# NSLab-CUK/LiteralKG

Measured on AMD Instinct MI355X. Metric: kg_edges_aggregated_per_sec, higher is better.
Workload: dtype f32

## Files before the change

literalkg_amd/_native.py:

```python
import ctypes as C
import os

_LIB_PATH = os.path.join(os.path.dirname(os.path.abspath(__file__)), "lib", "liblkg_hip.so")
_lib = None

i64, i32, f32, vp, u64 = C.c_int64, C.c_int32, C.c_float, C.c_void_p, C.c_uint64

PROTOTYPES = {
    "lkg_version": [],
    "lkg_last_error": [],
    "lkg_preload": [],
    "lkg_csr_build": [i64, i64, vp, vp, vp, vp, vp, vp, vp, vp, vp],
    "lkg_csr_transpose": [i64, i64, i64, vp, vp, vp, vp, vp],
    "lkg_row_partition": [i64, vp, i32, vp],
    "lkg_csr_coo_indices_i64": [i64, i64, vp, vp, vp, vp],
    "lkg_csr_build_device_workspace": [i64, i64],
    "lkg_csr_build_device": [i64, i64, vp, vp, vp, vp, vp, vp, vp, vp, vp, vp, i64, vp],
    "lkg_csr_transpose_device_workspace": [i64, i64],
    "lkg_csr_transpose_device": [i64, i64, i64, vp, vp, vp, vp, vp, vp, i64, vp],
    "lkg_triples_count": [C.c_char_p, vp],
    "lkg_triples_read": [C.c_char_p, i64, vp, vp, vp, vp],
    "lkg_triples_dedup": [i64, vp, vp, vp, vp, vp],
    "lkg_laplacian_f32": [i64, i64, i64, vp, vp, vp, vp, i32, vp],
    "lkg_laplacian_device_f32": [i64, i64, i32, vp, vp, vp, vp, i32, vp, vp, vp],
# ... 115 lines not shown
TRAIN_PROTOTYPES = {
    "lkg_nssa_fwd_f32": [i64, i64, i32, vp, i64, vp, i64, vp, i64, i32, f32, f32, f32, vp, vp, vp, vp, vp],
    "lkg_nssa_bwd_f32": [i64, i64, i32, vp, i64, vp, i64, vp, i64, i32, f32, vp, vp, vp, vp, vp, i64, vp, i64, vp, i64, vp],
}
SAMPLE_PROTOTYPES = {
    "lkg_sample_negatives": [i64, i64, u64, i64, vp, vp, vp, i64, i64, i32, i32, i32, vp, vp, vp, vp, vp, vp, vp, vp, vp, vp,
                             vp, i64, vp, i64, vp, vp, vp, vp],
    "lkg_relation_cardinality": [i64, i64, i64, vp, vp, vp, i64, vp, vp, vp, vp, vp, vp, vp],
    "lkg_answer_counts": [i64, vp, vp, vp, i64, vp, vp, vp, vp, vp, vp, vp, vp, vp],
}
RELATION_TRAIN_PROTOTYPES = {
    "lkg_relation_loss_fwd_f32": [i64, i32, i32, vp, i64, i64, vp, i64, vp, vp, vp, vp, vp, vp, vp, f32, vp, i64, vp, vp, vp],
    "lkg_relation_loss_bwd_f32": [i64, i32, i32, vp, i64, i64, vp, i64, vp, f32, vp, vp, i64, vp, i64, vp, i64, vp],
}
ORDERED_GEMM_PROTOTYPES = {
    "lkg_gemm_ordered_splits": [i32, i32, i64, i64, i64],
    "lkg_gemm_ordered_partition": [i64, i32, vp],
    "lkg_gemm_ordered_workspace": [i64, i64, i64, i32],
    "lkg_gemm_ordered_f32": [i32, i32, i64, i64, i64, i32, f32, vp, i64, vp, i64, f32, vp, i64, vp, vp, i64, vp],
}
NEIGHBOR_PROTOTYPES = {
    "lkg_csr_sample_rows": [i64, vp, vp, vp, vp, i32, u64, u64, i32, vp, vp, vp, vp],
}
_PAIR_ACCEPT_HEAD = [i64, i64, vp, vp, vp, vp, vp, vp, vp, vp, vp, vp, vp, vp, vp, vp, i32, vp]
PAIR_ACCEPT_PROTOTYPES = {
    "lkg_pair_mlp_accept_count_f32": _PAIR_ACCEPT_HEAD + [vp],
    "lkg_pair_mlp_accept_append_f32": _PAIR_ACCEPT_HEAD + [i64, vp, vp, vp, vp, vp],
    "lkg_pair_mlp_accept_emit_f32": _PAIR_ACCEPT_HEAD + [vp, vp, vp, vp, vp, vp, vp],
}
LIST_PROTOTYPES = {
    "lkg_list_scores_f32": [i64, i64, i64, i32, vp, i64, vp, vp, i64, vp, vp, i64, i32, vp, i64, vp],
    "lkg_list_count_f32": [i64, i64, i64, i32, vp, i64, vp, i64, vp, vp, i64, vp, vp, vp, vp, vp, vp, vp, vp, vp, vp, vp, vp],
}
_RESTYPE = {"lkg_last_error": C.c_char_p, "lkg_csr_build_device_workspace": C.c_int64,
            "lkg_gemm_tall_workspace": C.c_int64, "lkg_gemm_workspace": C.c_int64,
            "lkg_linear_act_layernorm_workspace": C.c_int64, "lkg_narrow_layer_bwd_workspace": C.c_int64,
            "lkg_csr_transpose_device_workspace": C.c_int64, "lkg_binary_curve_workspace": C.c_int64,
            "lkg_threshold_fit_workspace": C.c_int64, "lkg_accept_order_workspace": C.c_int64,
            "lkg_gemm_ordered_splits": C.c_int32, "lkg_gemm_ordered_partition": C.c_int64,
            "lkg_gemm_ordered_workspace": C.c_int64}


class LkgError(RuntimeError):
    pass


def lib_path():
    return _LIB_PATH


def load():
    global _lib
    if _lib is not None:
        return _lib
    if not os.path.exists(_LIB_PATH):
        raise LkgError(
            f"{_LIB_PATH} is missing: the HIP extension has not been built. Run "
            "`python -c 'import __graft_entry__ as g; g.build()'` (or `python -m literalkg_amd.build`). "
            "literalkg_amd has no CPU fallback.")
    lib = C.CDLL(_LIB_PATH)
    for name, argtypes in list(PROTOTYPES.items()) + list(EXTRA_PROTOTYPES.items()) + list(TRAIN_PROTOTYPES.items()) + \
            list(SAMPLE_PROTOTYPES.items()) + list(RELATION_TRAIN_PROTOTYPES.items()) + \
            list(ORDERED_GEMM_PROTOTYPES.items()) + list(NEIGHBOR_PROTOTYPES.items()) + \
            list(PAIR_ACCEPT_PROTOTYPES.items()) + list(LIST_PROTOTYPES.items()):
        fn = getattr(lib, name)
        fn.argtypes = argtypes
        fn.restype = _RESTYPE.get(name, C.c_int)
    _lib = lib
    return lib


_preloaded = False


def preload():
    global _preloaded
    if _preloaded:
        return
    import torch
    if not torch.cuda.is_initialized():
        return
    _preloaded = True
    lib = load()
    if lib.lkg_preload() != 0:
        msg = lib.lkg_last_error()
        raise LkgError(f"lkg_preload failed: {msg.decode() if msg else '?'}")


def call(name, *args):
    lib = load()
    if not _preloaded:
        preload()
    rc = getattr(lib, name)(*args)
    if rc != 0:
        msg = lib.lkg_last_error()
        raise LkgError(f"{name} failed ({rc}): {msg.decode() if msg else '?'}")

# ... 18 lines not shown
```

literalkg_amd/build.py:

```python
import hashlib
import os
import shutil
import subprocess
import sys
from concurrent.futures import ThreadPoolExecutor

HERE = os.path.dirname(os.path.abspath(__file__))
CSRC = os.path.join(HERE, "csrc")
LIB = os.path.join(HERE, "lib", "liblkg_hip.so")
OBJ = os.path.join(HERE, "lib", "obj")
SOURCES = ["lkg_graph_host.cpp", "lkg_spmm.hip", "lkg_attention.hip", "lkg_score.hip", "lkg_rowwise.hip",
           "lkg_gemm.hip", "lkg_batch.hip", "lkg_csr_device.hip", "lkg_gemm_tall.hip", "lkg_gemm_wgrad.hip", "lkg_layer.hip",
           "lkg_rank.hip", "lkg_topk.hip", "lkg_pairmlp.hip", "lkg_triples.hip", "lkg_relations.hip",
           "lkg_accept.hip", "lkg_retrieval.hip", "lkg_softmax.hip", "lkg_kvsall.hip", "lkg_nssa.hip", "lkg_negatives.hip",
           "lkg_relation_loss.hip", "lkg_gemm_ordered.hip", "lkg_neighbors.hip", "lkg_lists.hip"]
FLAGS = ["-O3", "--offload-arch=gfx950", "-fPIC", "-std=c++17"]


def _headers():
    return [os.path.join(CSRC, f) for f in sorted(os.listdir(CSRC)) if f.endswith(".h")] + \
           [os.path.join(HERE, "..", "include", h) for h in ("literalkg_hip.h", "literalkg_hip_ext.h", "literalkg_hip_train.h",
                                                                "literalkg_hip_sample.h", "literalkg_hip_relation_train.h",
                                                                "literalkg_hip_gemm_ordered.h", "literalkg_hip_neighbors.h",
                                                                "literalkg_hip_pair_accept.h", "literalkg_hip_lists.h")]


TAG_FILE = os.path.join(HERE, "lib", "flags.tag")


def _stale(tag):
    if not os.path.exists(LIB):
        return True
    if os.path.exists(TAG_FILE) and open(TAG_FILE).read().strip() != tag:
        return True
    t = os.path.getmtime(LIB)
    deps = [os.path.join(CSRC, f) for f in os.listdir(CSRC)] + _headers()
    return any(os.path.getmtime(d) > t for d in deps)


def _flag_tag(extra):
    return hashlib.sha256(" ".join(FLAGS + extra).encode()).hexdigest()[:12]


def build(force=False, verbose=True):
    extra = os.environ.get("LKG_EXTRA_HIPCC_FLAGS", "").split()
    tag = _flag_tag(extra)
    if not force and not _stale(tag):
        return LIB
    hipcc = shutil.which("hipcc") or "/opt/rocm/bin/hipcc"
    if not os.path.exists(hipcc):
        raise RuntimeError("hipcc not found: cannot build literalkg_amd/lib/liblkg_hip.so")
    os.makedirs(OBJ, exist_ok=True)
    newest_header = max(os.path.getmtime(h) for h in _headers())
    todo, objs = [], []
    for s in SOURCES:
        src = os.path.join(CSRC, s)
        obj = os.path.join(OBJ, f"{os.path.splitext(s)[0]}.{tag}.o")
# ... 27 lines not shown
```

literalkg_amd/csrc/lkg_graph_host.cpp:

```cpp
#include <fcntl.h>
#include <sys/mman.h>
#include <sys/stat.h>
#include <unistd.h>

#include <algorithm>
#include <atomic>
#include <cerrno>
#include <cmath>
#include <cstdlib>
#include <cstring>
#include <new>
#include <thread>
#include <vector>

#include "lkg_common.h"

static thread_local char g_err[512] = "";

void lkg_set_error(const char *fmt, ...) {
    va_list ap;
    va_start(ap, fmt);
    vsnprintf(g_err, sizeof(g_err), fmt, ap);
    va_end(ap);
}

extern "C" const char *lkg_last_error(void) { return g_err; }
extern "C" int lkg_version(void) { return 100;  }

int lkg_internal_preload_spmm();
int lkg_internal_preload_attention();
int lkg_internal_preload_batch();
int lkg_internal_preload_csr_device();
int lkg_internal_preload_gemm();
int lkg_internal_preload_gemm_tall();
int lkg_internal_preload_gemm_wgrad();
int lkg_internal_preload_rowwise();
int lkg_internal_preload_score();
int lkg_internal_preload_layer();
int lkg_internal_preload_rank();
int lkg_internal_preload_topk();
int lkg_internal_preload_pairmlp();
int lkg_internal_preload_triples();
int lkg_internal_preload_relations();
int lkg_internal_preload_accept();
int lkg_internal_preload_retrieval();
int lkg_internal_preload_softmax();
int lkg_internal_preload_kvsall();
int lkg_internal_preload_nssa();
int lkg_internal_preload_negatives();
int lkg_internal_preload_relation_loss();
int lkg_internal_preload_gemm_ordered();
int lkg_internal_preload_neighbors();
int lkg_internal_preload_lists();

extern "C" int lkg_preload(void) {
    const int failed = lkg_internal_preload_spmm() + lkg_internal_preload_attention() + lkg_internal_preload_batch() + lkg_internal_preload_csr_device() + lkg_internal_preload_gemm() + lkg_internal_preload_gemm_tall() + lkg_internal_preload_gemm_wgrad() + lkg_internal_preload_rowwise() + lkg_internal_preload_score() + lkg_internal_preload_layer() + lkg_internal_preload_rank() + lkg_internal_preload_topk() + lkg_internal_preload_pairmlp() + lkg_internal_preload_triples() + lkg_internal_preload_relations() + lkg_internal_preload_accept() + lkg_internal_preload_retrieval() + lkg_internal_preload_softmax() + lkg_internal_preload_kvsall() + lkg_internal_preload_nssa() + lkg_internal_preload_negatives() + lkg_internal_preload_relation_loss() + lkg_internal_preload_gemm_ordered() + lkg_internal_preload_neighbors() + lkg_internal_preload_lists();
    if (failed) {
        lkg_set_error("lkg_preload: %d of the library's code objects could not be loaded on the current device", failed);
        return LKG_ERR_HIP;
    }
    return LKG_OK;
}

namespace {
template <class F>
void parallel_rows(int64_t n, F &&fn) {
    unsigned hw = std::thread::hardware_concurrency();
    int nt = (int)std::min<int64_t>(std::max(1u, std::min(hw, 32u)), std::max<int64_t>(1, n / 65536));
    if (nt <= 1) {
        fn(0, n);
        return;
    }
    std::vector<std::thread> th;
    int64_t step = (n + nt - 1) / nt;
    for (int i = 0; i < nt; ++i) {
        int64_t lo = i * step, hi = std::min(n, lo + step);
        if (lo < hi) th.emplace_back([=, &fn] { fn(lo, hi); });
    }
    for (auto &x : th) x.join();
}
}

extern "C" int lkg_csr_build(int64_t n_entities, int64_t n_edges, const int64_t *h,
                             const int64_t *t, const int64_t *r, int32_t *rowptr, int32_t *col,
                             int32_t *eptr, int32_t *rel, int64_t *order, int64_t *nnz_out) {
    LKG_REQUIRE(n_entities >= 0 && n_entities < INT32_MAX, "lkg_csr_build: n_entities %lld out of int32 range",
                (long long)n_entities);
    LKG_REQUIRE(n_edges >= 0 && n_edges < INT32_MAX, "lkg_csr_build: n_edges %lld out of int32 range",
                (long long)n_edges);
// ... 383 lines not shown
```

literalkg_amd/model.py:

```python
from __future__ import annotations

import math
import os
from typing import Optional

import torch
import torch.nn as nn

from . import ops, pruned
from .gate import Gate, GateMul
from .graph import KGStructure


class AttentionCSR:

    def __init__(self, graph: KGStructure, val: torch.Tensor, val_t: Optional[torch.Tensor] = None):
        self.graph = graph
        self.val = val
        self.val_t = val_t if val_t is not None else (
            ops.permute_values(val, graph.t_perm) if graph.t_perm is not None and val.is_cuda else None)

    def aggregate(self, ego: torch.Tensor, plus_self: bool = False, bias: Optional[torch.Tensor] = None) -> torch.Tensor:
        return ops.aggregate(ego, self.graph, self.val, self.val_t, plus_self, bias)

# ... 123 lines not shown
    def narrows(self) -> bool:
        return self.aggregator_type == "gcn" and not self.use_residual and 2 * self.out_dim <= self.in_dim

    def forward(self, ego_embeddings, A_in: AttentionCSR, all_layers, lamda, alpha, l):
        ego = ego_embeddings
        h0 = all_layers[0]
        kind = self.aggregator_type
        if kind == "gcn":
            att = getattr(A_in, "att", A_in)
            if self.narrows() and isinstance(att, AttentionCSR):
                p = ops.linear(ego, self.linear.weight, None)
                return self._finish(att.aggregate(p, True, bias=self.linear.bias))
            if not self.use_residual:
                return self._linear_finish((A_in.aggregate(ego, True),), (self.linear.weight,), self.linear.bias)
            z = self._res_lin(self.linear, A_in.aggregate(ego, True), h0, lamda, alpha, l)
            return self._finish(z)
        if kind == "gin":
            return self._gin(ego, A_in.aggregate(ego, True), h0, all_layers, lamda, alpha, l)
        side = A_in.aggregate(ego)
        if kind == "graphsage":
            if self.use_residual:
                wh = self.linear_h.weight
                hi = ops.multi_linear((ego, side), (wh[:, :self.in_dim], wh[:, self.in_dim:]), self.linear_h.bias)
                z = self._res_lin(self.linear, hi, h0, lamda, alpha, l)
            else:
                w = self.linear.weight
                return self._linear_finish((ego, side), (w[:, :self.in_dim], w[:, self.in_dim:]), self.linear.bias)
            return self._finish(z)
        if kind == "bi-interaction":
            h0p = None
            if self.use_residual:
                h0p = self.h0_projection if self.h0_projection is not None else \
                    ops.linear(h0, self.linear_h0.weight, self.linear_h0.bias)
            ms, mp = ops.bi_mix(ego, side, h0p, alpha)
            if self.use_residual:
                wp = self._identity_map(lamda, l)
                s, b = self._lin_mapped(self.linear1, ms, wp), self._lin_mapped(self.linear2, mp, wp)
            else:
                s, b = self._lin(self.linear1, ms), self._lin(self.linear2, mp)
            return self._finish(ops.leaky_relu_sum(b, s), slope=1.0)
        raise NotImplementedError(kind)

    def _gin(self, ego, ego_plus_side, h0, all_layers, lamda, alpha, l):
        if self.num_layers == 1:
            raise AttributeError("gin with n_mlp_layers == 1 cannot run in the reference either "
                                 "(inp_linear/out_linear are never created, model.py:66-68, 133)")
        stack = self._lin(self.inp_linear, ego)
        h = self._lin(self.inp_linear, ego_plus_side)
        for lin, norm in zip(self.linears, self.mlp_layer_norms):
            h, _ = ops.act_layernorm(self._lin(lin, h), norm.weight, norm.bias, want_norm=False)
            stack = ops.axpby(stack, h)
        z = self._res_lin(self.out_linear, stack, h0, lamda, alpha, l)
        if len(all_layers) > 1:
            return self._finish(z, extra_sum=list(all_layers[1:]))
        return self._finish(z)


class LiteralKG(nn.Module):

    def __init__(self, args, n_entities, n_relations, A_in=None, numerical_literals=None, text_literals=None,
                 scoring: str = "transr"):
        super().__init__()
        if scoring not in ("transr", "transe"):
            raise ValueError(scoring)
        self.scoring = scoring
        self.args = args
# ... 593 lines not shown
```

literalkg_amd/ops.py:

```python
from __future__ import annotations

from typing import Optional, Sequence, Tuple

import torch
from torch.autograd import Function

from . import _native as N
from .graph import KGStructure, LONG_ROW_THRESHOLD

LEAKY_SLOPE = 0.01
LN_EPS = 1e-5
NORMALIZE_EPS = 1e-12


_raw_stream = getattr(torch._C, "_cuda_getCurrentRawStream", None)


def _stream():
    if _raw_stream is not None:
        return _raw_stream(torch.cuda.current_device())
    return torch.cuda.current_stream().cuda_stream


def _need_gpu(*ts):
# ... 1346 lines not shown
        rows_n, rows_y = tagged_rows(gyn), tagged_rows(gy)
        rows = union_rows(rows_y, rows_n) if (gy is None or rows_y is not None) and (gyn is None or rows_n is not None) else None
        gy_ = _f32_rows(gy) if gy is not None else None
        gyn_ = _f32_rows(gyn) if gyn is not None else None
        fused = (not rows_worth_compacting(rows, n) and need[0] and need[1] and gamma.data_ptr() % 16 == 0
                 and N.load().lkg_narrow_layer_bwd_ok(n, x.shape[1], d, N.ptr(x), _ld(x), N.ptr(z), _ld(z), N.ptr(y),
                                                      _ld(y) if y is not None else 0, N.ptr(gy_), _ld(gy_) if gy_ is not None else 0,
                                                      N.ptr(gyn_), _ld(gyn_) if gyn_ is not None else 0))
        if not fused:
            gz, gg, gb = _ActLayerNorm.backward(_ShimCtx((z, gamma, beta, mean, rstd, *kept_y), cfg=ctx.cfg), gy, gyn)[:3]
            lin = _MultiLinear.backward(_ShimCtx((x, w), n_terms=1, has_bias=ctx.has_bias,
                                                 needs_input_grad=(need[2], False, need[0], need[1])), gz)
            return (lin[2], lin[3], lin[0], gg, gb) + none[5:]
        gx = torch.empty((n, x.shape[1]), dtype=torch.float32, device=z.device)
        sums = torch.empty(32 * 32 + 3 * 32, dtype=torch.float32, device=z.device)
        gw, gbias, gg, gb = sums[:1024].view(32, 32), sums[1024:1056], sums[1056:1088], sums[1088:1120]
        wc = w if w.stride(1) == 1 else w.contiguous()
        ws_floats = int(N.load().lkg_narrow_layer_bwd_workspace(n))
        ws_ = _workspace(4 * ws_floats, z.device)
        N.call("lkg_narrow_layer_bwd_f32", n, x.shape[1], d, N.ptr(x), _ld(x), N.ptr(wc), _ld(wc), N.ptr(z), _ld(z), float(slope),
               N.ptr(gamma), N.ptr(y), _ld(y) if y is not None else 0, N.ptr(mean), N.ptr(rstd), N.ptr(gy_),
               _ld(gy_) if gy_ is not None else 0, N.ptr(gyn_), _ld(gyn_) if gyn_ is not None else 0, float(norm_eps), float(drop_p),
               int(seed), N.ptr(_flags(rows_n)) if gyn_ is not None else None, N.ptr(gx), _ld(gx), N.ptr(gw),
               N.ptr(gbias) if (ctx.has_bias and need[2]) else None, N.ptr(gg), N.ptr(gb), N.ptr(ws_), ws_floats, _stream())
        return (gx, gw, gbias if (ctx.has_bias and need[2]) else None, gg, gb) + none[5:]


def narrow_layer(x, w, bias, gamma, beta, want_norm=True, slope=LEAKY_SLOPE, eps=LN_EPS, norm_eps=NORMALIZE_EPS,
                 drop_p: float = 0.0, seed: Optional[int] = None, yn_out: Optional[torch.Tensor] = None, want_y: bool = True):
    if drop_p > 0 and seed is None:
        seed = new_seed()
    return _NarrowLayer.apply(x, w, bias, gamma, beta, want_norm, float(slope), float(eps), float(norm_eps), float(drop_p),
                              seed or 0, yn_out, want_y)


class CatBuffer:

    def __init__(self, n: int, widths: Sequence[int], device):
        self.widths = list(widths)
        self.offsets = [0]
        for w in self.widths:
            self.offsets.append(self.offsets[-1] + w)
        self.buf = torch.empty((n, self.offsets[-1]), dtype=torch.float32, device=device)

    def slot(self, k: int) -> torch.Tensor:
        return self.buf[:, self.offsets[k]:self.offsets[k + 1]]


def _same_view(a: torch.Tensor, b: torch.Tensor) -> bool:
    return (a.data_ptr() == b.data_ptr() and a.shape == b.shape
            and all(sa == sb for sa, sb, n_ in zip(a.stride(), b.stride(), a.shape) if n_ > 1))


class _AssembleCat(Function):
    @staticmethod
    def forward(ctx, holder: CatBuffer, pending, *parts):
        for k, p in enumerate(parts):
            s = holder.slot(k)
            if k in pending:
                continue
            if not _same_view(p, s):
                s.copy_(p)
        ctx.offsets = holder.offsets
        return holder.buf.detach()

    @staticmethod
# ... 1484 lines not shown
        pn = rank_sqnorm(p_) if distance else None
        exclude = (xptr, xcol) if xptr is not None else None
        lse, loss = softmax_all_forward(q_, p_, pn, truth, scale, splits, exclude)
        ctx.save_for_backward(q_, p_, pn, truth, lse, xptr, xcol)
        from .gemm_ordered import current_route
        ctx.route = current_route()
        ctx.meta = (scale, chunk_bytes)
        return loss

    @staticmethod
    def backward(ctx, g):
        q, p, pn, truth, lse, xptr, xcol = ctx.saved_tensors
        exclude = (xptr, xcol) if xptr is not None else None
        scale, chunk_bytes = ctx.meta
        want_q, want_p = ctx.needs_input_grad[0], ctx.needs_input_grad[1]
        g = g.reshape(-1).float().contiguous()

        def fill(c0, c1, out):
            return softmax_all_weights(q, p, pn, truth, lse, g, scale, c0, c1, out=out, exclude=exclude)

        width = softmax_chunk_width(q.shape[0], p.shape[0], chunk_bytes)
        return all_entity_backward(q, p, pn, width, want_q, want_p, fill, route=ctx.route) + (None,) * 7


def softmax_all_loss(q: torch.Tensor, p: torch.Tensor, truth: torch.Tensor, distance: bool = True, scale: float = 1.0,
                     splits: Optional[int] = None, chunk_bytes: int = SOFTMAX_CHUNK_BYTES, exclude=None,
                     products: str = "engine") -> torch.Tensor:
    from .gemm_ordered import keyword_route
    with keyword_route(products):
        _need_gpu(q, p, truth)
        scale, splits, chunk_bytes = check_softmax_args(scale, splits, chunk_bytes)
        xptr, xcol = list_pair("softmax_all_loss", "exclude", exclude, truth.numel())
        return _SoftmaxAllLoss.apply(q, p, truth, bool(distance), scale, splits, chunk_bytes, xptr, xcol)
```

Before: 6.597 billion.

## Fuse bi-interaction layer backward into a single HIP kernel

Adds a bi-interaction layer autograd Function whose backward runs the mix, both 32x32 linears, LeakyReLU, LayerNorm, dropout and the normalised-copy gradient in one kernel. Weight and LayerNorm gradient partials go to a workspace and are reduced by a second small kernel. This replaces roughly ten separate launches and the intermediate tensors they write and read back. The forward stays unfused but no longer materialises the mixed inputs for backward, so it recomputes them. The fused path only applies to 32-wide tensors with at least 4096 rows and aligned strides, and it adds a large new kernel that could be wrong or slow.

```diff
diff --git a/include/literalkg_hip_bi_layer.h b/include/literalkg_hip_bi_layer.h
--- /dev/null
+++ b/include/literalkg_hip_bi_layer.h
@@ -0,0 +1,30 @@
+#ifndef LITERALKG_HIP_BI_LAYER_H
+#define LITERALKG_HIP_BI_LAYER_H
+
+#include "literalkg_hip.h"
+
+#ifdef __cplusplus
+extern "C" {
+#endif
+
+int lkg_bi_layer_bwd_ok(int64_t n, int32_t d, const float *ego, int64_t ego_stride, const float *side, int64_t side_stride,
+                        const float *h0p, int64_t h0p_stride, const float *s, int64_t s_stride, const float *b, int64_t b_stride,
+                        const float *y, int64_t y_stride, const float *g_y, int64_t g_y_stride, const float *g_yn,
+                        int64_t g_yn_stride);
+
+int64_t lkg_bi_layer_bwd_workspace(int64_t n);
+
+int lkg_bi_layer_bwd_f32(int64_t n, int32_t d, const float *ego, int64_t ego_stride, const float *side, int64_t side_stride,
+                         const float *h0p, int64_t h0p_stride, float alpha, const float *w1, int64_t w1_stride, const float *w2,
+                         int64_t w2_stride, const float *s, int64_t s_stride, const float *b, int64_t b_stride, float slope,
+                         const float *gamma, const float *y, int64_t y_stride, const float *save_mean, const float *save_rstd,
+                         const float *g_y, int64_t g_y_stride, const float *g_yn, int64_t g_yn_stride, float norm_eps,
+                         float drop_p, uint64_t seed, const uint8_t *g_yn_rows, float *g_ego, float *g_side, float *g_h0p,
+                         float *g_w1, float *g_w2, float *g_b1, float *g_b2, float *g_gamma, float *g_beta, float *workspace,
+                         int64_t workspace_floats, void *stream);
+
+#ifdef __cplusplus
+}
+#endif
+
+#endif
diff --git a/literalkg_amd/_native.py b/literalkg_amd/_native.py
--- a/literalkg_amd/_native.py
+++ b/literalkg_amd/_native.py
@@ -171,13 +171,19 @@
     "lkg_list_scores_f32": [i64, i64, i64, i32, vp, i64, vp, vp, i64, vp, vp, i64, i32, vp, i64, vp],
     "lkg_list_count_f32": [i64, i64, i64, i32, vp, i64, vp, i64, vp, vp, i64, vp, vp, vp, vp, vp, vp, vp, vp, vp, vp, vp, vp],
 }
+BI_LAYER_PROTOTYPES = {
+    "lkg_bi_layer_bwd_ok": [i64, i32, vp, i64, vp, i64, vp, i64, vp, i64, vp, i64, vp, i64, vp, i64, vp, i64],
+    "lkg_bi_layer_bwd_workspace": [i64],
+    "lkg_bi_layer_bwd_f32": [i64, i32, vp, i64, vp, i64, vp, i64, f32, vp, i64, vp, i64, vp, i64, vp, i64, f32, vp, vp, i64, vp, vp,
+                             vp, i64, vp, i64, f32, f32, u64, vp, vp, vp, vp, vp, vp, vp, vp, vp, vp, vp, i64, vp],
+}
 _RESTYPE = {"lkg_last_error": C.c_char_p, "lkg_csr_build_device_workspace": C.c_int64,
             "lkg_gemm_tall_workspace": C.c_int64, "lkg_gemm_workspace": C.c_int64,
             "lkg_linear_act_layernorm_workspace": C.c_int64, "lkg_narrow_layer_bwd_workspace": C.c_int64,
             "lkg_csr_transpose_device_workspace": C.c_int64, "lkg_binary_curve_workspace": C.c_int64,
             "lkg_threshold_fit_workspace": C.c_int64, "lkg_accept_order_workspace": C.c_int64,
             "lkg_gemm_ordered_splits": C.c_int32, "lkg_gemm_ordered_partition": C.c_int64,
-            "lkg_gemm_ordered_workspace": C.c_int64}
+            "lkg_gemm_ordered_workspace": C.c_int64, "lkg_bi_layer_bwd_workspace": C.c_int64}
 
 
 class LkgError(RuntimeError):
@@ -201,7 +207,7 @@
     for name, argtypes in list(PROTOTYPES.items()) + list(EXTRA_PROTOTYPES.items()) + list(TRAIN_PROTOTYPES.items()) + \
             list(SAMPLE_PROTOTYPES.items()) + list(RELATION_TRAIN_PROTOTYPES.items()) + \
             list(ORDERED_GEMM_PROTOTYPES.items()) + list(NEIGHBOR_PROTOTYPES.items()) + \
-            list(PAIR_ACCEPT_PROTOTYPES.items()) + list(LIST_PROTOTYPES.items()):
+            list(PAIR_ACCEPT_PROTOTYPES.items()) + list(LIST_PROTOTYPES.items()) + list(BI_LAYER_PROTOTYPES.items()):
         fn = getattr(lib, name)
         fn.argtypes = argtypes
         fn.restype = _RESTYPE.get(name, C.c_int)
diff --git a/literalkg_amd/bi_layer.py b/literalkg_amd/bi_layer.py
--- /dev/null
+++ b/literalkg_amd/bi_layer.py
@@ -0,0 +1,140 @@
+from typing import Optional
+
+import torch
+from torch.autograd import Function
+
+from . import _native as N
+from . import ops as O
+
+
+class _NoSave:
+
+    def save_for_backward(self, *ts):
+        pass
+
+    def set_materialize_grads(self, flag):
+        pass
+
+
+def bi_layer_ok(ego: torch.Tensor, side: torch.Tensor, w1: torch.Tensor, w2: torch.Tensor,
+                h0p: Optional[torch.Tensor] = None) -> bool:
+    return (ego.is_cuda and ego.dim() == 2 and ego.shape[1] == 32 and ego.shape[0] >= 4096 and side.shape == ego.shape
+            and (h0p is None or h0p.shape == ego.shape) and tuple(w1.shape) == (32, 32) and tuple(w2.shape) == (32, 32)
+            and ego.dtype == torch.float32)
+
+
+def _mix(ego, side, h, alpha):
+    n, d = ego.shape
+    ms = torch.empty((n, d), dtype=torch.float32, device=ego.device)
+    mp = torch.empty((n, d), dtype=torch.float32, device=ego.device)
+    N.call("lkg_bi_mix_fwd_f32", n, d, N.ptr(ego), O._ld(ego), N.ptr(side), O._ld(side), N.ptr(h), O._ld(h) if h is not None else 0,
+           float(alpha), N.ptr(ms), d, N.ptr(mp), d, O._stream())
+    return ms, mp
+
+
+class _BiLayer(Function):
+
+    @staticmethod
+    def forward(ctx, ego, side, h0p, alpha, w1, b1, w2, b2, gamma, beta, want_norm, slope, eps, norm_eps, drop_p, seed, yn_out,
+                want_y):
+        O._need_gpu(ego, side, h0p, w1, w2, gamma, beta)
+        ego, side = O._f32_rows(ego), O._f32_rows(side)
+        h = O._f32_rows(h0p) if h0p is not None else None
+        if side.shape != ego.shape or (h is not None and h.shape != ego.shape):
+            raise ValueError("bi_layer: ego, side (and h0p) must have one shape")
+        if not want_y and not want_norm:
+            raise ValueError("bi_layer: neither output wanted")
+        n, d = ego.shape
+        ms, mp = _mix(ego, side, h, alpha)
+        s = O._MultiLinear.forward(_NoSave(), b1, 1, ms, w1)
+        b = O._MultiLinear.forward(_NoSave(), b2, 1, mp, w2)
+        u = O._elt(2, b, s, slope)
+        y = torch.empty((n, d), dtype=torch.float32, device=ego.device) if want_y else None
+        yn = None
+        if want_norm:
+            yn = yn_out if yn_out is not None else torch.empty((n, d), dtype=torch.float32, device=ego.device)
+        mean = torch.empty(n, dtype=torch.float32, device=ego.device)
+        rstd = torch.empty(n, dtype=torch.float32, device=ego.device)
+        N.call("lkg_act_layernorm_fwd_f32", n, d, N.ptr(u), O._ld(u), 1.0, N.ptr(gamma), N.ptr(beta), float(eps), N.ptr(y),
+               O._ld(y) if y is not None else 0, N.ptr(yn), O._ld(yn) if yn is not None else 0, float(norm_eps), N.ptr(mean),
+               N.ptr(rstd), float(drop_p), int(seed), O._stream())
+        ctx.save_for_backward(ego, side, w1, w2, s, b, gamma, beta, mean, rstd, *([h] if h is not None else []),
+                              *([y] if y is not None else []))
+        ctx.cfg = (h is not None, y is not None, float(alpha), slope, norm_eps, drop_p, seed, b1 is not None, b2 is not None)
+        ctx.set_materialize_grads(False)
+        return y, yn
+
+    @staticmethod
+    def backward(ctx, gy, gyn):
+        ego, side, w1, w2, s, b, gamma, beta, mean, rstd, *rest = ctx.saved_tensors
+        has_h, has_y, alpha, slope, norm_eps, drop_p, seed, has_b1, has_b2 = ctx.cfg
+        h = rest.pop(0) if has_h else None
+        y = rest.pop(0) if has_y else None
+        none = (None,) * 18
+        if gy is None and gyn is None:
+            return none
+        n, d = s.shape
+        need = ctx.needs_input_grad
+        need_b1, need_b2 = has_b1 and need[5], has_b2 and need[7]
+        rows_n, rows_y = O.tagged_rows(gyn), O.tagged_rows(gy)
+        rows = O.union_rows(rows_y, rows_n) if (gy is None or rows_y is not None) and (gyn is None or rows_n is not None) else None
+        gy_ = O._f32_rows(gy) if gy is not None else None
+        gyn_ = O._f32_rows(gyn) if gyn is not None else None
+
+        def ld(t):
+            return O._ld(t) if t is not None else 0
+        fused = (O.BI_LAYER_BWD and not O.rows_worth_compacting(rows, n) and need[0] and need[1] and (h is None or need[2])
+                 and need[4] and need[6] and gamma.data_ptr() % 16 == 0
+                 and bool(N.load().lkg_bi_layer_bwd_ok(n, d, N.ptr(ego), ld(ego), N.ptr(side), ld(side), N.ptr(h), ld(h), N.ptr(s), ld(s),
+                                                       N.ptr(b), ld(b), N.ptr(y), ld(y), N.ptr(gy_), ld(gy_), N.ptr(gyn_), ld(gyn_))))
+        if not fused:
+            return _BiLayer._unfused_backward(ctx, gy, gyn, ego, side, h, w1, w2, s, b, gamma, beta, mean, rstd, y) + none[10:]
+        dev = s.device
+        g_ego = torch.empty((n, d), dtype=torch.float32, device=dev)
+        g_side = torch.empty((n, d), dtype=torch.float32, device=dev)
+        g_h = torch.empty((n, d), dtype=torch.float32, device=dev) if h is not None else None
+        sums = torch.empty(2 * 32 * 32 + 4 * 32, dtype=torch.float32, device=dev)
+        gw1, gw2 = sums[:1024].view(32, 32), sums[1024:2048].view(32, 32)
+        gb1, gb2, gg, gb = sums[2048:2080], sums[2080:2112], sums[2112:2144], sums[2144:2176]
+        w1c = w1 if w1.stride(1) == 1 else w1.contiguous()
+        w2c = w2 if w2.stride(1) == 1 else w2.contiguous()
+        ws_floats = int(N.load().lkg_bi_layer_bwd_workspace(n))
+        ws_ = O._workspace(4 * ws_floats, dev)
+        N.call("lkg_bi_layer_bwd_f32", n, d, N.ptr(ego), ld(ego), N.ptr(side), ld(side), N.ptr(h), ld(h), float(alpha), N.ptr(w1c),
+               O._ld(w1c), N.ptr(w2c), O._ld(w2c), N.ptr(s), ld(s), N.ptr(b), ld(b), float(slope), N.ptr(gamma), N.ptr(y), ld(y),
+               N.ptr(mean), N.ptr(rstd), N.ptr(gy_), ld(gy_), N.ptr(gyn_), ld(gyn_), float(norm_eps), float(drop_p), int(seed),
+               N.ptr(O._flags(rows_n)) if gyn_ is not None else None, N.ptr(g_ego), N.ptr(g_side), N.ptr(g_h), N.ptr(gw1), N.ptr(gw2),
+               N.ptr(gb1) if need_b1 else None, N.ptr(gb2) if need_b2 else None, N.ptr(gg), N.ptr(gb), N.ptr(ws_), ws_floats,
+               O._stream())
+        return (g_ego, g_side, g_h, None, gw1, gb1 if need_b1 else None, gw2, gb2 if need_b2 else None, gg, gb) + none[10:]
+
+    @staticmethod
+    def _unfused_backward(ctx, gy, gyn, ego, side, h, w1, w2, s, b, gamma, beta, mean, rstd, y):
+        has_h, has_y, alpha, slope, norm_eps, drop_p, seed, has_b1, has_b2 = ctx.cfg
+        need = ctx.needs_input_grad
+        ms, mp = _mix(ego, side, h, alpha)
+        u = O._elt(2, b, s, slope)
+        gu, gg, gb = O._ActLayerNorm.backward(O._ShimCtx((u, gamma, beta, mean, rstd, *([y] if y is not None else [])),
+                                                         cfg=(1.0, norm_eps, drop_p, seed)), gy, gyn)[:3]
+        del u
+        g_b, g_s = O._LeakySum.backward(O._ShimCtx((b, s), slope=slope, needs_input_grad=(True, True, False)), gu)[:2]
+        del gu
+        need_x = need[0] or need[1] or (has_h and need[2])
+        lin1 = O._MultiLinear.backward(O._ShimCtx((ms, w1), n_terms=1, has_bias=has_b1,
+                                                  needs_input_grad=(has_b1 and need[5], False, need_x, need[4])), g_s)
+        lin2 = O._MultiLinear.backward(O._ShimCtx((mp, w2), n_terms=1, has_bias=has_b2,
+                                                  needs_input_grad=(has_b2 and need[7], False, need_x, need[6])), g_b)
+        g_ego = g_side = g_h = None
+        if need_x:
+            g_ego, g_side, g_h = O._BiMix.backward(O._ShimCtx((ego, side), cfg=(has_h, alpha)), lin1[2], lin2[2])[:3]
+        return (g_ego if need[0] else None, g_side if need[1] else None, g_h if (has_h and need[2]) else None, None,
+                lin1[3], lin1[0], lin2[3], lin2[0], gg, gb)
+
+
+def bi_layer(ego, side, h0p, alpha, w1, b1, w2, b2, gamma, beta, want_norm=True, slope=None, eps=None, norm_eps=None,
+             drop_p: float = 0.0, seed: Optional[int] = None, yn_out: Optional[torch.Tensor] = None, want_y: bool = True):
+    if drop_p > 0 and seed is None:
+        seed = O.new_seed()
+    return _BiLayer.apply(ego, side, h0p, float(alpha), w1, b1, w2, b2, gamma, beta, want_norm,
+                          float(O.LEAKY_SLOPE if slope is None else slope), float(O.LN_EPS if eps is None else eps),
+                          float(O.NORMALIZE_EPS if norm_eps is None else norm_eps), float(drop_p), seed or 0, yn_out, want_y)
diff --git a/literalkg_amd/build.py b/literalkg_amd/build.py
--- a/literalkg_amd/build.py
+++ b/literalkg_amd/build.py
@@ -13,7 +13,7 @@
            "lkg_gemm.hip", "lkg_batch.hip", "lkg_csr_device.hip", "lkg_gemm_tall.hip", "lkg_gemm_wgrad.hip", "lkg_layer.hip",
            "lkg_rank.hip", "lkg_topk.hip", "lkg_pairmlp.hip", "lkg_triples.hip", "lkg_relations.hip",
            "lkg_accept.hip", "lkg_retrieval.hip", "lkg_softmax.hip", "lkg_kvsall.hip", "lkg_nssa.hip", "lkg_negatives.hip",
-           "lkg_relation_loss.hip", "lkg_gemm_ordered.hip", "lkg_neighbors.hip", "lkg_lists.hip"]
+           "lkg_relation_loss.hip", "lkg_gemm_ordered.hip", "lkg_neighbors.hip", "lkg_lists.hip", "lkg_bi_layer.hip"]
 FLAGS = ["-O3", "--offload-arch=gfx950", "-fPIC", "-std=c++17"]
 
 
@@ -22,7 +22,8 @@
            [os.path.join(HERE, "..", "include", h) for h in ("literalkg_hip.h", "literalkg_hip_ext.h", "literalkg_hip_train.h",
                                                                 "literalkg_hip_sample.h", "literalkg_hip_relation_train.h",
                                                                 "literalkg_hip_gemm_ordered.h", "literalkg_hip_neighbors.h",
-                                                                "literalkg_hip_pair_accept.h", "literalkg_hip_lists.h")]
+                                                                "literalkg_hip_pair_accept.h", "literalkg_hip_lists.h",
+                                                                "literalkg_hip_bi_layer.h")]
 
 
 TAG_FILE = os.path.join(HERE, "lib", "flags.tag")
diff --git a/literalkg_amd/csrc/lkg_bi_layer.hip b/literalkg_amd/csrc/lkg_bi_layer.hip
--- /dev/null
+++ b/literalkg_amd/csrc/lkg_bi_layer.hip
@@ -0,0 +1,335 @@
+#include "lkg_common.h"
+
+#include "../../include/literalkg_hip_bi_layer.h"
+
+#include <algorithm>
+
+namespace {
+
+typedef float f32x16 __attribute__((ext_vector_type(16)));
+constexpr int D = 32;
+constexpr int LPR = 8;
+constexpr int RPP = 64 / LPR;
+constexpr int TILE = 32;
+constexpr int PITCH = 36;
+constexpr int WAVES = 4;
+constexpr int N_TILES = 4;
+constexpr int N_SUMS = 2 * D * D + 4 * D;
+constexpr int MAX_BLOCKS = 256 * 2;
+
+__global__ __launch_bounds__(256) __attribute__((amdgpu_waves_per_eu(2, 2))) void bi_layer_bwd_kernel(
+    long n, const float *__restrict__ ego, long lde, const float *__restrict__ side, long ldsd, const float *__restrict__ h0p, long ldh,
+    float alpha, const float *__restrict__ w1, long ldw1, const float *__restrict__ w2, long ldw2, const float *__restrict__ s,
+    long lds, const float *__restrict__ b, long ldb, float slope, const float *__restrict__ gamma, const float *__restrict__ y,
+    long ldy, const float *__restrict__ save_mean, const float *__restrict__ save_rstd, const float *__restrict__ g_y, long ldgy,
+    const float *__restrict__ g_yn, long ldgyn, float norm_eps, float drop_p, unsigned long long seed,
+    const unsigned char *__restrict__ gyn_rows, float *__restrict__ g_ego, float *__restrict__ g_side, float *__restrict__ g_h0p,
+    float *__restrict__ partials) {
+    __shared__ __attribute__((aligned(16))) float tiles[WAVES][N_TILES][TILE][PITCH];
+    const int lane = threadIdx.x & 63, wv = threadIdx.x >> 6, sl = lane % LPR, sub = lane / LPR;
+    const int e = sl * 4;
+    const int mm = lane & 31, kk = lane >> 5;
+    const long wave = (long)blockIdx.x * WAVES + wv, nwaves = (long)gridDim.x * WAVES;
+    const long n_tiles = (n + TILE - 1) / TILE;
+    const float c = h0p ? 1.f - alpha : 1.f;
+    float gam[4];
+    {
+        const float4 t = *reinterpret_cast<const float4 *>(gamma + e);
+        gam[0] = t.x; gam[1] = t.y; gam[2] = t.z; gam[3] = t.w;
+    }
+    float wb1[16], wb2[16];
+#pragma unroll
+    for (int t = 0; t < 16; ++t) {
+        wb1[t] = w1[(long)(2 * t + kk) * ldw1 + mm];
+        wb2[t] = w2[(long)(2 * t + kk) * ldw2 + mm];
+    }
+    f32x16 gw1_acc, gw2_acc;
+#pragma unroll
+    for (int r = 0; r < 16; ++r) gw1_acc[r] = gw2_acc[r] = 0.f;
+    float acc_g[4] = {0.f, 0.f, 0.f, 0.f}, acc_b[4] = {0.f, 0.f, 0.f, 0.f}, acc_b1[4] = {0.f, 0.f, 0.f, 0.f},
+          acc_b2[4] = {0.f, 0.f, 0.f, 0.f};
+    float(*gs_t)[PITCH] = tiles[wv][0];
+    float(*gb_t)[PITCH] = tiles[wv][1];
+    float(*ms_t)[PITCH] = tiles[wv][2];
+    float(*mp_t)[PITCH] = tiles[wv][3];
+
+    for (long tile = wave; tile < n_tiles; tile += nwaves) {
+        const long row0 = tile * TILE;
+#pragma unroll 2
+        for (int p = 0; p < TILE / RPP; ++p) {
+            const int tr = p * RPP + sub;
+            const long row_raw = row0 + tr;
+            const bool valid = row_raw < n;
+            const long row = valid ? row_raw : n - 1;
+            const bool has_gyn = g_yn && (!gyn_rows || gyn_rows[row]);
+            const bool any = valid && (g_y || has_gyn);
+            auto ld4 = [&](const float *base, long ld, bool on, float (&v)[4]) {
+                v[0] = v[1] = v[2] = v[3] = 0.f;
+                if (on) {
+                    const float4 t = *reinterpret_cast<const float4 *>(base + row * ld + e);
+                    v[0] = t.x; v[1] = t.y; v[2] = t.z; v[3] = t.w;
+                }
+            };
+            float sv[4], bv[4], G[4], ev[4], dv[4], hv[4];
+            ld4(s, lds, any, sv);
+            ld4(b, ldb, any, bv);
+            ld4(g_y, ldgy, any && g_y != nullptr, G);
+            ld4(ego, lde, any, ev);
+            ld4(side, ldsd, any, dv);
+            ld4(h0p, ldh, any && h0p != nullptr, hv);
+            {
+                float yy[4], gn[4];
+                ld4(y, ldy, any && has_gyn, yy);
+                ld4(g_yn, ldgyn, any && has_gyn, gn);
+                float n2 = 0.f, dt = 0.f;
+#pragma unroll
+                for (int k = 0; k < 4; ++k) {
+                    n2 = fmaf(yy[k], yy[k], n2);
+                    dt = fmaf(yy[k], gn[k], dt);
+                }
+                const float nrm = sqrtf(group_sum<LPR>(n2));
+                dt = group_sum<LPR>(dt);
+                if (nrm > norm_eps) {
+                    const float inv = 1.f / nrm;
+                    const float proj = dt * inv * inv * inv;
+#pragma unroll
+                    for (int k = 0; k < 4; ++k) G[k] += gn[k] * inv - yy[k] * proj;
+                } else {
+                    const float inv = 1.f / norm_eps;
+#pragma unroll
+                    for (int k = 0; k < 4; ++k) G[k] += gn[k] * inv;
+                }
+            }
+            if (drop_p > 0.f) {
+                const float inv_keep = 1.f / (1.f - drop_p);
+                const unsigned rkey = drop_row_key(seed, (unsigned long long)row);
+#pragma unroll
+                for (int k = 0; k < 4; ++k) G[k] *= drop_scale(rkey, (unsigned)(e + k), drop_p, inv_keep);
+            }
+            const float mean = save_mean[row], rstd = save_rstd[row];
+            float s1 = 0.f, s2 = 0.f, xh[4];
+#pragma unroll
+            for (int k = 0; k < 4; ++k) {
+                const float u = (bv[k] > 0.f ? bv[k] : slope * bv[k]) + (sv[k] > 0.f ? sv[k] : slope * sv[k]);
+                xh[k] = any ? (u - mean) * rstd : 0.f;
+                const float dx = G[k] * gam[k];
+                s1 += dx;
+                s2 = fmaf(dx, xh[k], s2);
+                acc_g[k] = fmaf(G[k], xh[k], acc_g[k]);
+                acc_b[k] += G[k];
+            }
+            s1 = group_sum<LPR>(s1) / (float)D;
+            s2 = group_sum<LPR>(s2) / (float)D;
+            float gs[4], gb[4], ms[4], mp[4];
+#pragma unroll
+            for (int k = 0; k < 4; ++k) {
+                const float dx = G[k] * gam[k];
+                const float da = rstd * (dx - s1 - xh[k] * s2);
+                const float gu = any ? da : 0.f;
+                gs[k] = gu * (sv[k] > 0.f ? 1.f : slope);
+                gb[k] = gu * (bv[k] > 0.f ? 1.f : slope);
+                acc_b1[k] += gs[k];
+                acc_b2[k] += gb[k];
+                const float hh = h0p ? alpha * hv[k] : 0.f;
+                ms[k] = fmaf(c, ev[k] + dv[k], hh);
+                mp[k] = fmaf(c, ev[k] * dv[k], hh);
+            }
+            *reinterpret_cast<float2 *>(&gs_t[tr][2 * sl]) = make_float2(gs[0], gs[2]);
+            *reinterpret_cast<float2 *>(&gs_t[tr][16 + 2 * sl]) = make_float2(gs[1], gs[3]);
+            *reinterpret_cast<float2 *>(&gb_t[tr][2 * sl]) = make_float2(gb[0], gb[2]);
+            *reinterpret_cast<float2 *>(&gb_t[tr][16 + 2 * sl]) = make_float2(gb[1], gb[3]);
+            *reinterpret_cast<float4 *>(&ms_t[tr][e]) = make_float4(ms[0], ms[1], ms[2], ms[3]);
+            *reinterpret_cast<float4 *>(&mp_t[tr][e]) = make_float4(mp[0], mp[1], mp[2], mp[3]);
+        }
+        __builtin_amdgcn_wave_barrier();
+        {
+            const int opos = (mm & 1) * 16 + (mm >> 1);
+#pragma unroll
+            for (int t = 0; t < 16; ++t) {
+                gw1_acc = __builtin_amdgcn_mfma_f32_32x32x2f32(gs_t[2 * t + kk][opos], ms_t[2 * t + kk][mm], gw1_acc, 0, 0, 0);
+                gw2_acc = __builtin_amdgcn_mfma_f32_32x32x2f32(gb_t[2 * t + kk][opos], mp_t[2 * t + kk][mm], gw2_acc, 0, 0, 0);
+            }
+        }
+        {
+            float ga[16], gc[16];
+#pragma unroll
+            for (int q = 0; q < 4; ++q) {
+                const float4 t4 = *reinterpret_cast<const float4 *>(&gs_t[mm][16 * kk + 4 * q]);
+                ga[4 * q] = t4.x; ga[4 * q + 1] = t4.y; ga[4 * q + 2] = t4.z; ga[4 * q + 3] = t4.w;
+                const float4 u4 = *reinterpret_cast<const float4 *>(&gb_t[mm][16 * kk + 4 * q]);
+                gc[4 * q] = u4.x; gc[4 * q + 1] = u4.y; gc[4 * q + 2] = u4.z; gc[4 * q + 3] = u4.w;
+            }
+            f32x16 gms, gmp;
+#pragma unroll
+            for (int r = 0; r < 16; ++r) gms[r] = gmp[r] = 0.f;
+#pragma unroll
+            for (int t = 0; t < 16; ++t) {
+                gms = __builtin_amdgcn_mfma_f32_32x32x2f32(ga[t], wb1[t], gms, 0, 0, 0);
+                gmp = __builtin_amdgcn_mfma_f32_32x32x2f32(gc[t], wb2[t], gmp, 0, 0, 0);
+            }
+            __builtin_amdgcn_wave_barrier();
+#pragma unroll
+            for (int r = 0; r < 16; ++r) {
+                const int tr = (r & 3) + 8 * (r >> 2) + 4 * kk;
+                gs_t[tr][mm] = gms[r];
+                gb_t[tr][mm] = gmp[r];
+            }
+        }
+        __builtin_amdgcn_wave_barrier();
+#pragma unroll
+        for (int p = 0; p < TILE / RPP; ++p) {
+            const int tr = p * RPP + sub;
+            const long row = row0 + tr;
+            if (row < n) {
+                const float4 e4 = *reinterpret_cast<const float4 *>(ego + row * lde + e);
+                const float4 d4 = *reinterpret_cast<const float4 *>(side + row * ldsd + e);
+                const float4 a4 = *reinterpret_cast<const float4 *>(&gs_t[tr][e]);
+                const float4 p4 = *reinterpret_cast<const float4 *>(&gb_t[tr][e]);
+                const float ev[4] = {e4.x, e4.y, e4.z, e4.w}, dv[4] = {d4.x, d4.y, d4.z, d4.w};
+                const float gsm[4] = {a4.x, a4.y, a4.z, a4.w}, gpr[4] = {p4.x, p4.y, p4.z, p4.w};
+                float ge[4], gd[4], gh[4];
+#pragma unroll
+                for (int k = 0; k < 4; ++k) {
+                    ge[k] = c * fmaf(gpr[k], dv[k], gsm[k]);
+                    gd[k] = c * fmaf(gpr[k], ev[k], gsm[k]);
+                    gh[k] = alpha * (gsm[k] + gpr[k]);
+                }
+                const long o = row * (long)D + e;
+                *reinterpret_cast<float4 *>(g_ego + o) = make_float4(ge[0], ge[1], ge[2], ge[3]);
+                *reinterpret_cast<float4 *>(g_side + o) = make_float4(gd[0], gd[1], gd[2], gd[3]);
+                if (g_h0p) *reinterpret_cast<float4 *>(g_h0p + o) = make_float4(gh[0], gh[1], gh[2], gh[3]);
+            }
+        }
+        __builtin_amdgcn_wave_barrier();
+    }
+
+#pragma unroll
+    for (int k = 0; k < 4; ++k) {
+        acc_g[k] = lane_xor_add<32>(lane_xor_add<16>(lane_xor_add<8>(acc_g[k])));
+        acc_b[k] = lane_xor_add<32>(lane_xor_add<16>(lane_xor_add<8>(acc_b[k])));
+        acc_b1[k] = lane_xor_add<32>(lane_xor_add<16>(lane_xor_add<8>(acc_b1[k])));
+        acc_b2[k] = lane_xor_add<32>(lane_xor_add<16>(lane_xor_add<8>(acc_b2[k])));
+    }
+    __syncthreads();
+    float *red_w = &tiles[0][0][0][0];
+    float *red_v = red_w + 3 * 32 * 64;
+    if (wv > 0) {
+#pragma unroll
+        for (int r = 0; r < 16; ++r) {
+            red_w[((wv - 1) * 32 + r) * 64 + lane] = gw1_acc[r];
+            red_w[((wv - 1) * 32 + 16 + r) * 64 + lane] = gw2_acc[r];
+        }
+        if (sub == 0) {
+#pragma unroll
+            for (int k = 0; k < 4; ++k) {
+                red_v[((wv - 1) * 4 + 0) * D + e + k] = acc_g[k];
+                red_v[((wv - 1) * 4 + 1) * D + e + k] = acc_b[k];
+                red_v[((wv - 1) * 4 + 2) * D + e + k] = acc_b1[k];
+                red_v[((wv - 1) * 4 + 3) * D + e + k] = acc_b2[k];
+            }
+        }
+    }
+    __syncthreads();
+    if (wv == 0) {
+        float *mine = partials + (long)blockIdx.x * N_SUMS;
+#pragma unroll
+        for (int r = 0; r < 16; ++r) {
+            const int o = (r & 3) + 8 * (r >> 2) + 4 * kk;
+            mine[o * D + mm] = gw1_acc[r] + red_w[(0 * 32 + r) * 64 + lane] + red_w[(1 * 32 + r) * 64 + lane] + red_w[(2 * 32 + r) * 64 + lane];
+            mine[D * D + o * D + mm] = gw2_acc[r] + red_w[(0 * 32 + 16 + r) * 64 + lane] + red_w[(1 * 32 + 16 + r) * 64 + lane] +
+                                       red_w[(2 * 32 + 16 + r) * 64 + lane];
+        }
+        if (sub == 0) {
+            auto fold = [&](int q, const float (&acc)[4]) {
+#pragma unroll
+                for (int k = 0; k < 4; ++k)
+                    mine[2 * D * D + q * D + e + k] = acc[k] + red_v[(0 * 4 + q) * D + e + k] + red_v[(1 * 4 + q) * D + e + k] +
+                                                      red_v[(2 * 4 + q) * D + e + k];
+            };
+            fold(0, acc_g);
+            fold(1, acc_b);
+            fold(2, acc_b1);
+            fold(3, acc_b2);
+        }
+    }
+}
+
+__global__ __launch_bounds__(1024) void bi_layer_sums_kernel(const float *__restrict__ partials, int rows, float *__restrict__ g_w1,
+                                                             float *__restrict__ g_w2, float *__restrict__ g_gamma,
+                                                             float *__restrict__ g_beta, float *__restrict__ g_b1,
+                                                             float *__restrict__ g_b2) {
+    __shared__ float red[32][33];
+    const int c = blockIdx.x * 32 + (threadIdx.x & 31), slice = threadIdx.x >> 5;
+    float v = 0.f;
+    for (int r = slice; r < rows; r += 32) v += partials[(long)r * N_SUMS + c];
+    red[slice][threadIdx.x & 31] = v;
+    __syncthreads();
+    if (slice == 0) {
+        float t = 0.f;
+#pragma unroll
+        for (int q = 0; q < 32; ++q) t += red[q][threadIdx.x & 31];
+        if (c < D * D) g_w1[c] = t;
+        else if (c < 2 * D * D) g_w2[c - D * D] = t;
+        else if (c < 2 * D * D + D) g_gamma[c - 2 * D * D] = t;
+        else if (c < 2 * D * D + 2 * D) g_beta[c - 2 * D * D - D] = t;
+        else if (c < 2 * D * D + 3 * D) { if (g_b1) g_b1[c - 2 * D * D - 2 * D] = t; }
+        else if (g_b2) g_b2[c - 2 * D * D - 3 * D] = t;
+    }
+}
+
+}
+
+extern "C" int lkg_bi_layer_bwd_ok(int64_t n, int32_t d, const float *ego, int64_t ego_stride, const float *side, int64_t side_stride,
+                                   const float *h0p, int64_t h0p_stride, const float *s, int64_t s_stride, const float *b,
+                                   int64_t b_stride, const float *y, int64_t y_stride, const float *g_y, int64_t g_y_stride,
+                                   const float *g_yn, int64_t g_yn_stride) {
+    auto rows_ok = [](const float *p, int64_t ld) { return !p || (ld >= D && ld % 4 == 0 && lkg_aligned16(p)); };
+    return n >= 4096 && d == D && ego && side && s && b && rows_ok(ego, ego_stride) && rows_ok(side, side_stride) &&
+           rows_ok(h0p, h0p_stride) && rows_ok(s, s_stride) && rows_ok(b, b_stride) && rows_ok(y, y_stride) &&
+           rows_ok(g_y, g_y_stride) && rows_ok(g_yn, g_yn_stride) && (g_y || g_yn) && (!g_yn || y);
+}
+
+extern "C" int64_t lkg_bi_layer_bwd_workspace(int64_t n) {
+    const int64_t tiles = (std::max<int64_t>(n, 0) + TILE - 1) / TILE;
+    return std::max<int64_t>(1, std::min<int64_t>((tiles + WAVES - 1) / WAVES, MAX_BLOCKS)) * N_SUMS;
+}
+
+extern "C" int lkg_bi_layer_bwd_f32(int64_t n, int32_t d, const float *ego, int64_t ego_stride, const float *side, int64_t side_stride,
+                                    const float *h0p, int64_t h0p_stride, float alpha, const float *w1, int64_t w1_stride,
+                                    const float *w2, int64_t w2_stride, const float *s, int64_t s_stride, const float *b,
+                                    int64_t b_stride, float slope, const float *gamma, const float *y, int64_t y_stride,
+                                    const float *save_mean, const float *save_rstd, const float *g_y, int64_t g_y_stride,
+                                    const float *g_yn, int64_t g_yn_stride, float norm_eps, float drop_p, uint64_t seed,
+                                    const uint8_t *g_yn_rows, float *g_ego, float *g_side, float *g_h0p, float *g_w1, float *g_w2,
+                                    float *g_b1, float *g_b2, float *g_gamma, float *g_beta, float *workspace,
+                                    int64_t workspace_floats, void *stream) {
+    LKG_REQUIRE(n >= 0 && d > 0 && workspace_floats >= 0, "lkg_bi_layer_bwd_f32: negative size");
+    if (n == 0) return LKG_OK;
+    LKG_REQUIRE(ego && side && w1 && w2 && s && b && gamma && save_mean && save_rstd && g_ego && g_side && g_w1 && g_w2 && g_gamma &&
+                g_beta && (g_y || g_yn) && workspace && (!h0p || g_h0p), "lkg_bi_layer_bwd_f32: null pointer");
+    LKG_REQUIRE(w1_stride >= d && w2_stride >= d, "lkg_bi_layer_bwd_f32: a weight's row stride is shorter than its row");
+    LKG_REQUIRE(lkg_bi_layer_bwd_ok(n, d, ego, ego_stride, side, side_stride, h0p, h0p_stride, s, s_stride, b, b_stride, y, y_stride, g_y,
+                                    g_y_stride, g_yn, g_yn_stride) && lkg_aligned16(g_ego) && lkg_aligned16(g_side) &&
+                (!g_h0p || lkg_aligned16(g_h0p)) && lkg_aligned16(gamma),
+                "lkg_bi_layer_bwd_f32: needs 32 columns, n >= 4096, 16-byte aligned rows of at least 32 floats and y wherever g_yn is "
+                "given (lkg_bi_layer_bwd_ok)");
+    LKG_REQUIRE(drop_p >= 0.f && drop_p < 1.f, "lkg_bi_layer_bwd_f32: drop_p outside [0, 1)");
+    LKG_REQUIRE(workspace_floats >= lkg_bi_layer_bwd_workspace(n), "lkg_bi_layer_bwd_f32: workspace of %lld floats, %lld needed "
+                "(lkg_bi_layer_bwd_workspace)", (long long)workspace_floats, (long long)lkg_bi_layer_bwd_workspace(n));
+    hipStream_t st = (hipStream_t)stream;
+    const unsigned blocks = (unsigned)(lkg_bi_layer_bwd_workspace(n) / N_SUMS);
+    hipLaunchKernelGGL(bi_layer_bwd_kernel, dim3(blocks), dim3(256), 0, st, (long)n, ego, (long)ego_stride, side, (long)side_stride, h0p,
+                       (long)h0p_stride, alpha, w1, (long)w1_stride, w2, (long)w2_stride, s, (long)s_stride, b, (long)b_stride, slope,
+                       gamma, y, (long)y_stride, save_mean, save_rstd, g_y, (long)g_y_stride, g_yn, (long)g_yn_stride, norm_eps, drop_p,
+                       (unsigned long long)seed, g_yn_rows, g_ego, g_side, h0p ? g_h0p : nullptr, workspace);
+    LKG_CHECK_LAUNCH("lkg_bi_layer_bwd_f32");
+    hipLaunchKernelGGL(bi_layer_sums_kernel, dim3(N_SUMS / 32), dim3(1024), 0, st, workspace, (int)blocks, g_w1, g_w2, g_gamma, g_beta,
+                       g_b1, g_b2);
+    LKG_CHECK_LAUNCH("lkg_bi_layer_bwd_f32 (sums)");
+    return LKG_OK;
+}
+
+int lkg_internal_preload_bi_layer() {
+    hipFuncAttributes attr;
+    return hipFuncGetAttributes(&attr, reinterpret_cast<const void *>(&bi_layer_bwd_kernel)) == hipSuccess ? 0 : 1;
+}
diff --git a/literalkg_amd/csrc/lkg_graph_host.cpp b/literalkg_amd/csrc/lkg_graph_host.cpp
--- a/literalkg_amd/csrc/lkg_graph_host.cpp
+++ b/literalkg_amd/csrc/lkg_graph_host.cpp
@@ -52,9 +52,10 @@
 int lkg_internal_preload_gemm_ordered();
 int lkg_internal_preload_neighbors();
 int lkg_internal_preload_lists();
+int lkg_internal_preload_bi_layer();
 
 extern "C" int lkg_preload(void) {
-    const int failed = lkg_internal_preload_spmm() + lkg_internal_preload_attention() + lkg_internal_preload_batch() + lkg_internal_preload_csr_device() + lkg_internal_preload_gemm() + lkg_internal_preload_gemm_tall() + lkg_internal_preload_gemm_wgrad() + lkg_internal_preload_rowwise() + lkg_internal_preload_score() + lkg_internal_preload_layer() + lkg_internal_preload_rank() + lkg_internal_preload_topk() + lkg_internal_preload_pairmlp() + lkg_internal_preload_triples() + lkg_internal_preload_relations() + lkg_internal_preload_accept() + lkg_internal_preload_retrieval() + lkg_internal_preload_softmax() + lkg_internal_preload_kvsall() + lkg_internal_preload_nssa() + lkg_internal_preload_negatives() + lkg_internal_preload_relation_loss() + lkg_internal_preload_gemm_ordered() + lkg_internal_preload_neighbors() + lkg_internal_preload_lists();
+    const int failed = lkg_internal_preload_spmm() + lkg_internal_preload_attention() + lkg_internal_preload_batch() + lkg_internal_preload_csr_device() + lkg_internal_preload_gemm() + lkg_internal_preload_gemm_tall() + lkg_internal_preload_gemm_wgrad() + lkg_internal_preload_rowwise() + lkg_internal_preload_score() + lkg_internal_preload_layer() + lkg_internal_preload_rank() + lkg_internal_preload_topk() + lkg_internal_preload_pairmlp() + lkg_internal_preload_triples() + lkg_internal_preload_relations() + lkg_internal_preload_accept() + lkg_internal_preload_retrieval() + lkg_internal_preload_softmax() + lkg_internal_preload_kvsall() + lkg_internal_preload_nssa() + lkg_internal_preload_negatives() + lkg_internal_preload_relation_loss() + lkg_internal_preload_gemm_ordered() + lkg_internal_preload_neighbors() + lkg_internal_preload_lists() + lkg_internal_preload_bi_layer();
     if (failed) {
         lkg_set_error("lkg_preload: %d of the library's code objects could not be loaded on the current device", failed);
         return LKG_ERR_HIP;
diff --git a/literalkg_amd/model.py b/literalkg_amd/model.py
--- a/literalkg_amd/model.py
+++ b/literalkg_amd/model.py
@@ -179,6 +179,18 @@
             if self.use_residual:
                 h0p = self.h0_projection if self.h0_projection is not None else \
                     ops.linear(h0, self.linear_h0.weight, self.linear_h0.bias)
+            if ego.is_cuda and not self.reference_association and \
+                    ops.bi_layer_ok(ego, side, self.linear1.weight, self.linear2.weight, h0p):
+                w1, w2 = self.linear1.weight, self.linear2.weight
+                if self.use_residual:
+                    wp = self._identity_map(lamda, l)
+                    w1, w2 = ops.fold_nt(w1, wp), ops.fold_nt(w2, wp)
+                ln = self.layer_normalize
+                y, yn = ops.bi_layer(ego, side, h0p, alpha, w1, self.linear1.bias, w2, self.linear2.bias, ln.weight, ln.bias,
+                                     want_norm=True, drop_p=float(self.dropout) if self.training else 0.0,
+                                     yn_out=self.norm_out, want_y=self.want_output)
+                self.last_normalized = yn
+                return y
             ms, mp = ops.bi_mix(ego, side, h0p, alpha)
             if self.use_residual:
                 wp = self._identity_map(lamda, l)
diff --git a/literalkg_amd/ops.py b/literalkg_amd/ops.py
--- a/literalkg_amd/ops.py
+++ b/literalkg_amd/ops.py
@@ -1402,6 +1402,13 @@
         seed = new_seed()
     return _NarrowLayer.apply(x, w, bias, gamma, beta, want_norm, float(slope), float(eps), float(norm_eps), float(drop_p),
                               seed or 0, yn_out, want_y)
+
+
+BI_LAYER_BWD = True
+"""Run the DENSE backward of a 32 -> 32 bi-interaction layer (the mix, both Linears, both LeakyReLUs, LayerNorm, dropout and the
+normalised copy) as one launch (lkg_bi_layer_bwd_f32) instead of about ten.  False: _BiLayer always runs the unfused passes' own
+backward (tests and tools/bi_layer_micro.py run both).  The Function lives in bi_layer.py and is re-exported at the end of this
+module; the forward launches are the unfused ones either way."""
 
 
 class CatBuffer:
@@ -2952,3 +2959,6 @@
         scale, splits, chunk_bytes = check_softmax_args(scale, splits, chunk_bytes)
         xptr, xcol = list_pair("softmax_all_loss", "exclude", exclude, truth.numel())
         return _SoftmaxAllLoss.apply(q, p, truth, bool(distance), scale, splits, chunk_bytes, xptr, xcol)
+
+
+from .bi_layer import _BiLayer, bi_layer, bi_layer_ok
```

New measurement: 6.595 billion. About the same (-0.0%).
